# kaspanet/rusty-kaspa

Measured on NVIDIA H100. Metric: schnorr_sig_verifies_per_sec, higher is better.
Workload: dtype u32 limbs (256-bit modular integer)

## Files before the change

### __graft_entry__.py

```python
import os
import subprocess
import sys

ROOT = os.path.dirname(os.path.abspath(__file__))
CSRC = os.path.join(ROOT, "rusty_kaspa_b200", "csrc")
LIB = os.path.join(ROOT, "rusty_kaspa_b200", "libkgv.so")
NVCC_FLAGS = ["-gencode", "arch=compute_90a,code=sm_90a", "-O3", "-lineinfo", "-std=c++17", "-shared", "-Xcompiler", "-fPIC"]


def _newer(target, sources):
    if not os.path.exists(target):
        return True
    t = os.path.getmtime(target)
    return any(os.path.getmtime(s) > t for s in sources)


def _run(cmd, **kw):
    r = subprocess.run(cmd, capture_output=True, text=True, **kw)
    if r.returncode != 0:
        raise RuntimeError("command failed: %s\n%s\n%s" % (" ".join(cmd), r.stdout[-4000:], r.stderr[-4000:]))
    return r


def build():
    srcs = [os.path.join(d, f) for d, _, fs in os.walk(CSRC) for f in fs] + [os.path.join(ROOT, "include", "kgv.h")]
    units = sorted(s for s in srcs if s.endswith(".cu") or s.endswith(".cpp"))
    if _newer(LIB, srcs):
        nvcc = os.environ.get("NVCC", "nvcc")
        _run([nvcc] + NVCC_FLAGS + ["-o", LIB] + units)
    _run(["make", "-C", os.path.join(ROOT, "oracle")])
    hs = os.path.join(ROOT, "tests", "hostsim")
    for name in ("hostsim_arith", "hostsim_secp", "hostsim_comb", "hostsim_joint", "hostsim_hash", "hostsim_u3072", "hostsim_script", "hostsim_standard"):
        src, out = os.path.join(hs, name + ".cpp"), os.path.join(hs, "lib" + name + ".so")
        if os.path.exists(src) and _newer(out, [src] + srcs):
            _run(["g++", "-O2", "-std=c++17", "-shared", "-fPIC", "-o", out, src])
    sg_src, sg_lib = os.path.join(ROOT, "tools", "simgen", "kgv_simgen.cpp"), os.path.join(ROOT, "tools", "simgen", "libkgv_simgen.so")
    if os.path.exists(sg_src) and _newer(sg_lib, [sg_src]):
        _run(["g++", "-O2", "-std=c++17", "-shared", "-fPIC", "-o", sg_lib, sg_src])
    for name in ("host_mirror_test", "script_engine_mirror_test"):
        cpp_src, cpp_bin = os.path.join(ROOT, "tests", "cpp", name + ".cpp"), os.path.join(ROOT, "tests", "cpp", name)
        if os.path.exists(cpp_src) and _newer(cpp_bin, [cpp_src, LIB, os.path.join(ROOT, "include", "kgv.hpp"), os.path.join(ROOT, "include", "kgv.h")]):
            _run(["g++", "-O2", "-std=c++17", "-o", cpp_bin, cpp_src, "-L" + os.path.join(ROOT, "rusty_kaspa_b200"), "-l:libkgv.so", "-Wl,-rpath,$ORIGIN/../../rusty_kaspa_b200"])
    sys.path.insert(0, ROOT)
    import rusty_kaspa_b200
    from rusty_kaspa_b200 import _lib
    _lib.load()


def smoke():
    import ctypes
    import numpy as np
    sys.path.insert(0, ROOT)
    import rusty_kaspa_b200 as rk
    from rusty_kaspa_b200 import workload as W
    pk, msg, sig, kind = W.schnorr_triples(4096, seed=7, n_keys=256, n_nonces=256, frac_bitflip=0.05, frac_adversarial=0.05)
    ctx = rk.GpuContext(0)
    got = ctx.verify_schnorr_batch(pk, msg, sig)
    ora = ctypes.CDLL(os.path.join(ROOT, "oracle", "libkaspa_oracle.so"))
    ora.ok_secp_init()
    exp = np.zeros(len(pk), dtype=np.uint8)
    vp = lambda a: a.ctypes.data_as(ctypes.c_void_p)
    ora.ok_schnorr_verify_batch(vp(pk), vp(msg), vp(sig), ctypes.c_size_t(len(pk)), vp(exp), 4)
    assert (got == exp).all(), "GPU verdicts differ from the oracle"
    assert (got[kind == 0] == 1).all() and not (got[kind != 0] == 1).any()
    bm = ctx.status_to_bitmap(got)
    assert (bm == np.packbits((got == 1).astype(np.uint8), bitorder="little")).all()
    sys.path.insert(0, os.path.join(ROOT, "tests"))
    from rusty_kaspa_b200 import simgen
    from rusty_kaspa_b200.txbatch import build_batch
    from rusty_kaspa_b200.validator import TransactionValidator, Params
    import oracle_tx
    fk, fe, txs = simgen.funded_window(96, n_keys=64, n_nonces=64, mix=(0.5, 0.2, 0.15, 0.15))
    ents, k = [], 0
    for t in txs:
        ents.append(fe[k:k + len(t["inputs"])])
        k += len(t["inputs"])
    txs[5]["inputs"][0]["sigscript"] = txs[5]["inputs"][0]["sigscript"][:10] + bytes([txs[5]["inputs"][0]["sigscript"][10] ^ 1]) + txs[5]["inputs"][0]["sigscript"][11:]
    batch = build_batch(txs, ents)
    val = TransactionValidator(ctx, Params(storage_mass_parameter=simgen.DEFAULT_STORAGE_MASS_PARAMETER))
    res = val.validate_populated_transactions(batch, pov_daa_score=10)
    op = oracle_tx.params(coinbase_maturity=100, storage_mass_parameter=simgen.DEFAULT_STORAGE_MASS_PARAMETER)
    for i in range(len(txs)):
        e = oracle_tx.validate_populated(ora, batch, i, 10, 0, op)
        assert int(res["status"][i]) == int(e["status"]) and int(res["fee"][i]) == int(e["fee"]), (i, res[i], e)
    assert int(res["status"][5]) != 0
    from rusty_kaspa_b200.replay import DagReplayer, REPLAY_BLOCK_DTYPE
    g = simgen.FastDag(seed=3, n_keys=64, n_nonces=128, coinbase_maturity=3, mix=(0.5, 0.2, 0.15, 0.15), frac_invalid=0.1, coinbase_outputs=8)
    g.generate(24, 12)
    b, first, pov = g.take()
    arr = np.zeros(len(pov), dtype=REPLAY_BLOCK_DTYPE)
    arr["first_tx"], arr["n_txs"], arr["pov_daa_score"], arr["flags"] = first[:-1], np.diff(first), pov, 1
    rp = DagReplayer(ctx, Params(coinbase_maturity=3, storage_mass_parameter=g.C), 1 << 12)
    got_r, acc = rp.replay_window(b, arr, want_accept=True)
    ost = oracle_tx.State(ora)
    exp_r, eacc = oracle_tx.state_replay(ost, b, first, pov, oracle_tx.params(coinbase_maturity=3, storage_mass_parameter=g.C), threads=2)
    assert (got_r["status"] == exp_r["status"]).all() and (got_r["script_err"] == exp_r["script_err"]).all() and (acc == eacc).all(), "replay verdicts differ from the oracle"
    assert rp.us.count() == ost.count() and rp.us.digest() == ost.digest()
    n_replayed = len(b.txs)
    rp.close(); ost.close(); g.close()
    ctx.close()
    print("smoke ok: %d triples (%d valid), %d transactions and a replay window of %d transactions, verdicts identical to the oracle"
          % (len(pk), int((got == 1).sum()), len(txs), n_replayed))


if __name__ == "__main__":
    build()
    print("build ok")
```

### rusty_kaspa_b200/csrc/kgv_lib.cu

```cuda
#include "../../include/kgv.h"
#include "kgv_internal.h"
#include "kgv_verify.cuh"
#include "kgv_lanes.cuh"

#include <cuda_runtime.h>
#include <cstdio>
#include <algorithm>
#include <cstring>
#include <mutex>
#include <string>

using namespace kgv;

struct SmemTab {
  uint32_t* base;
  __device__ __forceinline__ void put(int e, int w, uint32_t v) { base[(e * 16 + w) * KGV_BLOCK] = v; }
  __device__ __forceinline__ uint32_t get(int e, int w) const { return base[(e * 16 + w) * KGV_BLOCK]; }
  __device__ __forceinline__ uint4* chunk(int q) const { return reinterpret_cast<uint4*>(base - threadIdx.x) + q * KGV_BLOCK + threadIdx.x; }
};
__device__ __forceinline__ void stage_fetch(SmemTab& tab, int s, const uint32_t* entry) {
#pragma unroll
  for (int c = 0; c < 4; c++) {
    const uint32_t dst = (uint32_t)__cvta_generic_to_shared(tab.chunk(4 * s + c));
    asm volatile("cp.async.cg.shared.global [%0], [%1], 16;" ::"r"(dst), "l"(entry + 4 * c) : "memory");
// ... 1 lines not shown
}
__device__ __forceinline__ void stage_commit(SmemTab&) { asm volatile("cp.async.commit_group;" ::: "memory"); }
__device__ __forceinline__ void stage_wait(SmemTab&) { asm volatile("cp.async.wait_group 7;" ::: "memory"); }
__device__ __forceinline__ void stage_get(SmemTab& tab, int s, fe& x, fe& y) {
  const uint4 a = *tab.chunk(4 * s), b = *tab.chunk(4 * s + 1), c = *tab.chunk(4 * s + 2), d = *tab.chunk(4 * s + 3);
  x.v[0] = a.x; x.v[1] = a.y; x.v[2] = a.z; x.v[3] = a.w; x.v[4] = b.x; x.v[5] = b.y; x.v[6] = b.z; x.v[7] = b.w;
  y.v[0] = c.x; y.v[1] = c.y; y.v[2] = c.z; y.v[3] = c.w; y.v[4] = d.x; y.v[5] = d.y; y.v[6] = d.z; y.v[7] = d.w;
}

__device__ __forceinline__ void ldg256(uint32_t* w, const void* p) {
  asm volatile("ld.global.nc.v4.u32 {%0,%1,%2,%3}, [%8];\n\t"
               "ld.global.nc.v4.u32 {%4,%5,%6,%7}, [%8+16];"
               : "=r"(w[0]), "=r"(w[1]), "=r"(w[2]), "=r"(w[3]), "=r"(w[4]), "=r"(w[5]), "=r"(w[6]), "=r"(w[7])
               : "l"(p));
}
__device__ __forceinline__ void ldg256_stream(uint32_t* w, const void* p) {
  asm volatile("ld.global.nc.L1::no_allocate.v4.u32 {%0,%1,%2,%3}, [%8];\n\t"
               "ld.global.nc.L1::no_allocate.v4.u32 {%4,%5,%6,%7}, [%8+16];"
               : "=r"(w[0]), "=r"(w[1]), "=r"(w[2]), "=r"(w[3]), "=r"(w[4]), "=r"(w[5]), "=r"(w[6]), "=r"(w[7])
               : "l"(p));
}

struct GLoadDev {
  __device__ __forceinline__ void operator()(fe& x, fe& y, const uint32_t* entry) const {
    ldg256(x.v, entry);
    ldg256(y.v, entry + 8);
  }
};

template <bool ALIGNED>
__device__ __forceinline__ void load_be32(uint32_t* w, const uint8_t* p) {
  if (ALIGNED) {
    ldg256_stream(w, p);
#pragma unroll
    for (int i = 0; i < 8; i++) w[i] = bswap32(w[i]);
  } else {
#pragma unroll
    for (int i = 0; i < 8; i++)
      w[i] = ((uint32_t)p[4 * i] << 24) | ((uint32_t)p[4 * i + 1] << 16) | ((uint32_t)p[4 * i + 2] << 8) | (uint32_t)p[4 * i + 3];
  }
}

__global__ void __launch_bounds__(128) k_build_gtab(uint32_t* __restrict__ gtab) {
  uint32_t t = blockIdx.x * blockDim.x + threadIdx.x;
  if (t >= 8u * 65536u) return;
  uint32_t v = t & 0xFFFFu;
  uint32_t which = t >> 16;
  uint32_t* out = gtab + (size_t)t * 16;
  if (v == 0) {
#pragma unroll
    for (int i = 0; i < 16; i++) out[i] = 0;
    return;
  }
  fe bx, by, x, y;
  gtab_base(bx, by, (int)which);
  gtab_entry(x, y, v, bx, by);
#pragma unroll
  for (int i = 0; i < 8; i++) { out[i] = x.v[i]; out[8 + i] = y.v[i]; }
}

#define KGV_KEY_RECORDS_MAX (1u << 17)
#ifndef KGV_COMB_USES
#define KGV_COMB_USES 8
#endif
enum { KGV_KEYS_INLINE = 0, KGV_KEYS_PLAIN = 1, KGV_KEYS_COMB = 2 };
__host__ __device__ __forceinline__ int key_form(uint32_t n_rec, size_t n) {
  if (n_rec > KGV_KEY_RECORDS_MAX || 2 * (size_t)n_rec > n) return KGV_KEYS_INLINE;
  return (size_t)KGV_COMB_USES * n_rec <= n ? KGV_KEYS_COMB : KGV_KEYS_PLAIN;
}

struct KeySlot {
  unsigned long long key;
  uint32_t rec, unused_;
};
struct KeyCacheView {
  const KeySlot* table;
  const uint32_t* item_slot;
  const uint32_t* recs;
  const uint32_t* n_rec;
  __device__ __forceinline__ KeySrc key_of(size_t i, size_t n) const {
    const int f = n_rec ? key_form(*n_rec, n) : KGV_KEYS_INLINE;
    if (f == KGV_KEYS_INLINE) return KeySrc{nullptr, false};
    const bool comb = f == KGV_KEYS_COMB;
    return KeySrc{recs + (size_t)(table[item_slot[i]].rec - 1) * (comb ? KGV_KJ_WORDS : KGV_KR_WORDS), comb};
  }
};

template <bool ALIGNED, bool ECDSA>
__device__ __forceinline__ void key_words(uint32_t* w, const uint8_t* pk, size_t i) {
  if (ECDSA) {
    const uint8_t* kp = pk + 33 * i;
    w[8] = kp[0];
    load_be32<false>(w, kp + 1);
  } else {
    load_be32<ALIGNED>(w, pk + 32 * i);
  }
}
__device__ __forceinline__ uint64_t key_hash(const uint32_t* w, int nw) {
  uint64_t h = 0x9E3779B97F4A7C15ull;
  for (int k = 0; k < nw; k++) {
    h = (h ^ w[k]) * 0xFF51AFD7ED558CCDull;
    h ^= h >> 32;
  }
  h ^= h >> 33; h *= 0xC4CEB9FE1A85EC53ull; h ^= h >> 33;
  return h;
}

template <bool ALIGNED, bool ECDSA>
__global__ void __launch_bounds__(256) k_key_dedup(const uint8_t* __restrict__ pk, size_t n_arg, const uint32_t* __restrict__ index,
                                                   const uint32_t* __restrict__ n_dev, KeySlot* __restrict__ table, uint32_t mask,
                                                   uint32_t* __restrict__ item_slot, uint32_t* __restrict__ rec_rep, uint32_t* n_rec) {
  const size_t n = n_dev ? (size_t)*n_dev : n_arg;
  const size_t t = (size_t)blockIdx.x * blockDim.x + threadIdx.x;
  if (t >= n || key_form(*(volatile uint32_t*)n_rec, n) == KGV_KEYS_INLINE) return;
  const size_t i = index ? index[t] : t;
  const int nw = ECDSA ? 9 : 8;
  uint32_t w[9];
  key_words<ALIGNED, ECDSA>(w, pk, i);
  const uint64_t h = key_hash(w, nw);
  const unsigned long long mine = (h & 0xFFFFFFFF00000000ull) | (uint64_t)(i + 1);
  uint32_t s = (uint32_t)h & mask;
  bool won = false;
  for (;;) {
    unsigned long long cur = atomicCAS(&table[s].key, 0ull, mine);
    if (cur == 0) { won = true; break; }
    if ((cur >> 32) == (mine >> 32)) {
      uint32_t v[9];
      key_words<ALIGNED, ECDSA>(v, pk, (uint32_t)cur - 1);
      bool eq = true;
      for (int k = 0; k < nw; k++) eq = eq && v[k] == w[k];
      if (eq) break;
    }
    s = (s + 1) & mask;
  }
  const uint32_t act = __activemask(), ball = __ballot_sync(act, won);
  const int lane = threadIdx.x & 31, leader = __ffs(act) - 1;
  uint32_t base = 0;
  if (lane == leader && ball) base = atomicAdd(n_rec, (uint32_t)__popc(ball));
  base = __shfl_sync(act, base, leader);
  if (won) {
    const uint32_t r = base + __popc(ball & ((1u << lane) - 1));
    if (key_form(r + 1, n) != KGV_KEYS_INLINE) {
      rec_rep[r] = (uint32_t)i;
      table[s].rec = r + 1;
    }
  }
  item_slot[i] = s;
}

template <bool ECDSA>
__global__ void __launch_bounds__(KGV_BLOCK, KGV_BLOCKS_PER_SM) k_key_prepare(const uint8_t* __restrict__ pk, size_t n_arg, const uint32_t* __restrict__ n_dev,
                                                                              const uint32_t* __restrict__ rec_rep, const uint32_t* __restrict__ n_rec,
                                                                              uint32_t* __restrict__ recs) {
  const size_t n = n_dev ? (size_t)*n_dev : n_arg;
  const uint32_t r = blockIdx.x * blockDim.x + threadIdx.x;
  const int f = key_form(*n_rec, n);
  if (r >= *n_rec || f == KGV_KEYS_INLINE) return;
  uint32_t w[9];
  key_words<false, ECDSA>(w, pk, rec_rep[r]);
  if (f == KGV_KEYS_COMB) {
    uint32_t* rec = recs + (size_t)r * KGV_KJ_WORDS;
    key_comb_build(rec, ECDSA ? w[8] : 2u, w);
    if (rec[KGV_KC_STATUS] == KGV_ST_VALID) key_joint_build(rec);
  } else key_rec_build(recs + (size_t)r * KGV_KR_WORDS, ECDSA ? w[8] : 2u, w);
}

template <bool ECDSA>
__device__ __forceinline__ void batch_mul(fe& r, const fe& a, const fe& b) {
  if constexpr (ECDSA) sc_mul(r.v, a.v, b.v);
  else fe_mul(r, a, b);
}
template <bool ECDSA, bool ALIGNED, bool INDEXED>
__device__ __forceinline__ void verify_body(const uint8_t* __restrict__ pk, const uint8_t* __restrict__ msg, const uint8_t* __restrict__ sig,
                                            size_t n_arg, uint8_t* __restrict__ status, const uint32_t* __restrict__ gtab,
                                            const uint32_t* __restrict__ index, const uint32_t* __restrict__ n_dev, KeyCacheView kc) {
  extern __shared__ uint32_t smem[];
  const size_t n = (INDEXED && n_dev) ? (size_t)*n_dev : n_arg;
  const size_t total = (size_t)gridDim.x * KGV_BLOCK;
  const size_t tid = (size_t)blockIdx.x * KGV_BLOCK + threadIdx.x;
  SmemTab tab{smem + threadIdx.x};
  fe X[KGV_ITEMS], Y[KGV_ITEMS], RX[KGV_ITEMS], D[KGV_ITEMS], pre[KGV_ITEMS], M[KGV_ITEMS];
  const uint32_t* KR[KGV_ITEMS];
  bool comb = false;
  uint8_t st[KGV_ITEMS];
#pragma unroll 1
  for (size_t base = 0; base < n; base += total * KGV_ITEMS) {
  fe acc;
  fe_set_u32(acc, 1);
  bool any = false;
#pragma unroll 1
  for (int j = 0; j < KGV_ITEMS; j++) {
    size_t i = base + tid + (size_t)j * total;
    st[j] = KGV_ST_INVALID;
    if (i >= n) continue;
    if (INDEXED) i = index[i];
    uint32_t pkw[9], mw[8], sw[16];
    key_words<ALIGNED, ECDSA>(pkw, pk, i);
    load_be32<ALIGNED>(mw, msg + 32 * i);
    load_be32<ALIGNED>(sw, sig + 64 * i);
    load_be32<ALIGNED>(sw + 8, sig + 64 * i + 32);
    const KeySrc key = kc.key_of(i, n);
    fe x, y, rx, d, m;
    uint8_t s1;
    if constexpr (ECDSA) s1 = ecdsa_phase1(x, y, rx.v, d.v, m.v, pkw[8], pkw, mw, sw, key);
    else s1 = schnorr_phase1(x, y, d, rx, pkw, mw, sw, tab, gtab, GLoadDev(), key);
    st[j] = s1;
    if (s1 == KGV_ST_PENDING) {
      X[j] = x; Y[j] = y; RX[j] = rx; D[j] = d;
      if constexpr (ECDSA) { M[j] = m; KR[j] = key.rec; comb = key.comb; }
      pre[j] = acc;
      batch_mul<ECDSA>(acc, acc, d);
      any = true;
    }
  }
  if (any) {
    fe inv;
    if constexpr (ECDSA) sc_inv(inv.v, acc.v);
    else fe_inv(inv, acc);
#pragma unroll 1
    for (int j = KGV_ITEMS - 1; j >= 0; j--) {
      if (st[j] != KGV_ST_PENDING) continue;
      fe di;
      batch_mul<ECDSA>(di, inv, pre[j]);
      batch_mul<ECDSA>(inv, inv, D[j]);
      if constexpr (ECDSA) st[j] = ecdsa_phase2(X[j], Y[j], RX[j].v, di.v, M[j].v, tab, gtab, GLoadDev(), KeySrc{KR[j], comb});
      else st[j] = schnorr_phase2(X[j], Y[j], di, RX[j]);
    }
  }
#pragma unroll 1
  for (int j = 0; j < KGV_ITEMS; j++) {
    size_t i = base + tid + (size_t)j * total;
    if (i < n) status[INDEXED ? index[i] : i] = st[j];
  }
  }
}

template <bool ALIGNED, bool INDEXED>
__global__ void __launch_bounds__(KGV_BLOCK, KGV_BLOCKS_PER_SM)
k_schnorr_verify(const uint8_t* __restrict__ pk, const uint8_t* __restrict__ msg, const uint8_t* __restrict__ sig, size_t n_arg,
                 uint8_t* __restrict__ status, const uint32_t* __restrict__ gtab, const uint32_t* __restrict__ index, const uint32_t* __restrict__ n_dev,
                 KeyCacheView kc) {
  verify_body<false, ALIGNED, INDEXED>(pk, msg, sig, n_arg, status, gtab, index, n_dev, kc);
}
template <bool ALIGNED, bool INDEXED>
__global__ void __launch_bounds__(KGV_BLOCK, KGV_BLOCKS_PER_SM)
k_ecdsa_verify(const uint8_t* __restrict__ pk, const uint8_t* __restrict__ msg, const uint8_t* __restrict__ sig, size_t n_arg,
               uint8_t* __restrict__ status, const uint32_t* __restrict__ gtab, const uint32_t* __restrict__ index, const uint32_t* __restrict__ n_dev,
// ... 153 lines not shown
    k_build_gtab<<<(8 * 65536) / 128, 128, 0, ctx->stream>>>(ctx->gtab);
    CK(cudaGetLastError());
    ctx->launches++;
    const int smem = KGV_BLOCK * 128 * (int)sizeof(uint32_t);
    for (const auto& kind : k_verify)
      for (const auto& form : kind)
        for (VerifyKernel k : form) CK(cudaFuncSetAttribute(k, cudaFuncAttributeMaxDynamicSharedMemorySize, smem));
    int per_sm = 0, sms = 0;
    CK(cudaOccupancyMaxActiveBlocksPerMultiprocessor(&per_sm, k_verify[0][0][1], KGV_BLOCK, smem));
    CK(cudaDeviceGetAttribute(&sms, cudaDevAttrMultiProcessorCount, device));
    ctx->resident_blocks = per_sm * sms > 0 ? per_sm * sms : 132 * KGV_BLOCKS_PER_SM;
    CK(cudaStreamSynchronize(ctx->stream));
    return KGV_OK;
  };
  int rc = body();
  if (rc != KGV_OK) {
    fprintf(stderr, "kgv_create: %s\n", ctx->err.c_str());
    delete ctx;
    return rc;
  }
  *out = ctx;
  return KGV_OK;
}

extern "C" void kgv_destroy(kgv_ctx* ctx) {
  if (!ctx) return;
  cudaSetDevice(ctx->device);
  for (auto& P : ctx->prefetch) if (P.worker.joinable()) P.worker.join();
  if (ctx->copy_stream) cudaStreamSynchronize(ctx->copy_stream);
  cudaStreamSynchronize(ctx->stream);
  if (ctx->gtab) cudaFree(ctx->gtab);
  for (uint8_t* b : {ctx->d_in, ctx->d_out, ctx->d_batch, ctx->prefetch[0].buf, ctx->prefetch[1].buf, ctx->d_scratch, ctx->d_mu, ctx->d_work, ctx->d_replay, ctx->d_keys[0], ctx->d_keys[1]})
    if (b) cudaFree(b);
  for (uint8_t* b : ctx->parked) cudaFree(b);
  for (cudaEvent_t e : ctx->ev_chunk) if (e) cudaEventDestroy(e);
  for (cudaEvent_t e : ctx->ev_time) if (e) cudaEventDestroy(e);
  if (ctx->ev_prefetch) cudaEventDestroy(ctx->ev_prefetch);
  for (auto& P : ctx->prefetch) if (P.done) cudaEventDestroy(P.done);
  if (ctx->copy_stream) cudaStreamDestroy(ctx->copy_stream);
  if (ctx->ev_fork) cudaEventDestroy(ctx->ev_fork);
  if (ctx->ev_join) cudaEventDestroy(ctx->ev_join);
  if (ctx->aux_stream) cudaStreamDestroy(ctx->aux_stream);
  if (ctx->own_stream) cudaStreamDestroy(ctx->own_stream);
  delete ctx;
}

extern "C" int kgv_set_stream(kgv_ctx* ctx, void* cuda_stream) {
  if (!ctx) return KGV_ERR_ARG;
  std::lock_guard<std::recursive_mutex> g(ctx->mu);
  ctx->stream = (cudaStream_t)cuda_stream;
  return KGV_OK;
}

extern "C" int kgv_reset_stream(kgv_ctx* ctx) {
  if (!ctx) return KGV_ERR_ARG;
  std::lock_guard<std::recursive_mutex> g(ctx->mu);
  ctx->stream = ctx->own_stream;
  return KGV_OK;
}

extern "C" int kgv_synchronize(kgv_ctx* ctx) {
  if (!ctx) return KGV_ERR_ARG;
  std::lock_guard<std::recursive_mutex> g(ctx->mu);
  CK(cudaSetDevice(ctx->device));
  CK(cudaStreamSynchronize(ctx->stream));
  if (!ctx->parked.empty()) {
    CK(cudaStreamSynchronize(ctx->aux_stream));
    if (ctx->copy_stream) CK(cudaStreamSynchronize(ctx->copy_stream));
    for (uint8_t* p : ctx->parked) cudaFree(p);
    ctx->parked.clear();
  }
  return KGV_OK;
}

extern "C" const char* kgv_last_error(const kgv_ctx* ctx) { return ctx ? ctx->err.c_str() : "null context"; }
extern "C" uint64_t kgv_launch_count(const kgv_ctx* ctx) { return ctx ? ctx->launches : 0; }

static int key_cache_launch(kgv_ctx* ctx, const uint8_t* dpk, size_t n, bool ecdsa, bool aligned, cudaStream_t st, const uint32_t* index,
                            const uint32_t* n_dev, KeyCacheView* kc) {
  uint32_t slots = 64;
  while (slots < 2 * n) slots <<= 1;
  const uint32_t cap = (uint32_t)(n / 2 < KGV_KEY_RECORDS_MAX ? n / 2 : KGV_KEY_RECORDS_MAX);
  const size_t cap_comb = n / KGV_COMB_USES < KGV_KEY_RECORDS_MAX ? n / KGV_COMB_USES : KGV_KEY_RECORDS_MAX;
  const size_t rec_bytes = std::max((size_t)cap * KGV_KR_WORDS, cap_comb * KGV_KJ_WORDS) * 4;
  const size_t o_tab = 256, o_item = o_tab + (size_t)slots * sizeof(KeySlot);
  const size_t o_rep = (o_item + n * 4 + 255) & ~(size_t)255, o_rec = (o_rep + (size_t)cap * 4 + 255) & ~(size_t)255;
  int rc = kgv_reserve(ctx, &ctx->d_keys[ecdsa], &ctx->d_keys_cap[ecdsa], o_rec + rec_bytes);
  if (rc) return rc;
  uint8_t* K = ctx->d_keys[ecdsa];
  uint32_t* n_rec = (uint32_t*)K;
  KeySlot* table = (KeySlot*)(K + o_tab);
  uint32_t *item_slot = (uint32_t*)(K + o_item), *rec_rep = (uint32_t*)(K + o_rep), *recs = (uint32_t*)(K + o_rec);
  CK(cudaMemsetAsync(K, 0, o_item, st));
  const unsigned gd = (unsigned)((n + 255) / 256);
  const auto dedup = ecdsa ? k_key_dedup<false, true> : aligned ? k_key_dedup<true, false> : k_key_dedup<false, false>;
  dedup<<<gd, 256, 0, st>>>(dpk, n, index, n_dev, table, slots - 1, item_slot, rec_rep, n_rec);
  CK(cudaGetLastError());
  ctx->launches++;
  if (cap) {
    const unsigned gp = (cap + KGV_BLOCK - 1) / KGV_BLOCK;
    const auto prepare = ecdsa ? k_key_prepare<true> : k_key_prepare<false>;
    prepare<<<gp, KGV_BLOCK, 0, st>>>(dpk, n, n_dev, rec_rep, n_rec, recs);
    CK(cudaGetLastError());
    ctx->launches++;
  }
  *kc = KeyCacheView{table, item_slot, recs, n_rec};
  return KGV_OK;
}

int kgv_launch_verify(kgv_ctx* ctx, const uint8_t* dpk, const uint8_t* dmsg, const uint8_t* dsig, size_t n, uint8_t* dst, bool ecdsa,
                      cudaStream_t st, const uint32_t* index, const uint32_t* n_dev) {
  if (n == 0) return KGV_OK;
  if (n >= 0x7FFFFFFFu) return fail_arg(ctx, "verify launch of 2^31 or more items");
  const int smem = KGV_BLOCK * 128 * (int)sizeof(uint32_t);
  size_t want = (n + KGV_BLOCK - 1) / KGV_BLOCK;
  unsigned blocks = (unsigned)(want < (size_t)ctx->resident_blocks ? want : (size_t)ctx->resident_blocks);
  bool aligned = (((uintptr_t)dmsg | (uintptr_t)dsig | (ecdsa ? 0 : (uintptr_t)dpk)) & 31) == 0;
  KeyCacheView kc{};
  const bool key_cache = n > (size_t)ctx->resident_blocks * KGV_BLOCK;
  if (key_cache) {
    int rc = key_cache_launch(ctx, dpk, n, ecdsa, aligned, st, index, n_dev, &kc);
    if (rc) return rc;
  }
  if (!index) {
    auto& lv = ctx->last_verify[ecdsa];
    lv.n = n; lv.blocks = blocks; lv.key_cache = key_cache; lv.stream = st;
  }
  k_verify[ecdsa][index != nullptr][aligned]<<<blocks, KGV_BLOCK, smem, st>>>(dpk, dmsg, dsig, n, dst, ctx->gtab, index, n_dev, kc);
  CK(cudaGetLastError());
  ctx->launches++;
  return KGV_OK;
}

static int verify_common(kgv_ctx* ctx, const uint8_t* pk, size_t pk_stride, const uint8_t* msg, const uint8_t* sig, size_t n,
                         uint8_t* status, bool ecdsa) {
  if (!ctx) return KGV_ERR_ARG;
  std::lock_guard<std::recursive_mutex> g(ctx->mu);
  if (n == 0) return KGV_OK;
  if (!pk || !msg || !sig || !status) return fail_arg(ctx, "null buffer");
  CK(cudaSetDevice(ctx->device));
  int dev = kgv_ptr_is_device(pk);
  if (kgv_ptr_is_device(msg) != dev || kgv_ptr_is_device(sig) != dev || kgv_ptr_is_device(status) != dev)
    return fail_arg(ctx, "all buffers of one call must be host pointers or all device pointers");
  const uint8_t *dpk = pk, *dmsg = msg, *dsig = sig;
  uint8_t* dst = status;
  if (!dev) {
    size_t off_msg = (pk_stride * n + 255) & ~(size_t)255;
    size_t off_sig = off_msg + 32 * n;
    int rc = kgv_reserve(ctx, &ctx->d_in, &ctx->d_in_cap, off_sig + 64 * n);
    if (rc) return rc;
    rc = kgv_reserve(ctx, &ctx->d_out, &ctx->d_out_cap, n);
    if (rc) return rc;
    dpk = ctx->d_in; dmsg = ctx->d_in + off_msg; dsig = ctx->d_in + off_sig; dst = ctx->d_out;
    const size_t chunk = (size_t)ctx->resident_blocks * KGV_BLOCK * KGV_ITEMS;
    if (n >= 2 * chunk && (n + chunk - 1) / chunk <= 32) {
      CK(cudaEventRecord(ctx->ev_fork, ctx->stream));
      CK(cudaStreamWaitEvent(ctx->aux_stream, ctx->ev_fork, 0));
      size_t c = 0;
      for (size_t a = 0; a < n; a += chunk, c++) {
        const size_t m = n - a < chunk ? n - a : chunk;
        if (!ctx->ev_chunk[c]) CK(cudaEventCreateWithFlags(&ctx->ev_chunk[c], cudaEventDisableTiming));
        CK(cudaMemcpyAsync(ctx->d_in + pk_stride * a, pk + pk_stride * a, pk_stride * m, cudaMemcpyHostToDevice, ctx->aux_stream));
        CK(cudaMemcpyAsync(ctx->d_in + off_msg + 32 * a, msg + 32 * a, 32 * m, cudaMemcpyHostToDevice, ctx->aux_stream));
        CK(cudaMemcpyAsync(ctx->d_in + off_sig + 64 * a, sig + 64 * a, 64 * m, cudaMemcpyHostToDevice, ctx->aux_stream));
        CK(cudaEventRecord(ctx->ev_chunk[c], ctx->aux_stream));
        CK(cudaStreamWaitEvent(ctx->stream, ctx->ev_chunk[c], 0));
        int rc2 = kgv_launch_verify(ctx, dpk + pk_stride * a, dmsg + 32 * a, dsig + 64 * a, m, dst + a, ecdsa, ctx->stream);
// ... 144 lines not shown
```

### rusty_kaspa_b200/csrc/kgv_secp.cuh

```cuda
#pragma once
#include "kgv_arith.cuh"

namespace kgv {

#define KGV_N_LIMBS {0xD0364141u, 0xBFD25E8Cu, 0xAF48A03Bu, 0xBAAEDCE6u, 0xFFFFFFFEu, 0xFFFFFFFFu, 0xFFFFFFFFu, 0xFFFFFFFFu}
#define KGV_BETA_LIMBS {0x719501EEu, 0xC1396C28u, 0x12F58995u, 0x9CF04975u, 0xAC3434E9u, 0x6E64479Eu, 0x657C0710u, 0x7AE96A2Bu}
#define KGV_G1_LIMBS {0x45DBB031u, 0xE893209Au, 0x71E8CA7Fu, 0x3DAA8A14u, 0x9284EB15u, 0xE86C90E4u, 0xA7D46BCDu, 0x3086D221u}
#define KGV_G2_LIMBS {0x8AC47F71u, 0x1571B4AEu, 0x9DF506C6u, 0x221208ACu, 0x0ABFE4C4u, 0x6F547FA9u, 0x010E8828u, 0xE4437ED6u}
#define KGV_A1_LIMBS {0x9284EB15u, 0xE86C90E4u, 0xA7D46BCDu, 0x3086D221u, 0u}
#define KGV_MB1_LIMBS {0x0ABFE4C3u, 0x6F547FA9u, 0x010E8828u, 0xE4437ED6u, 0u}
#define KGV_A2_LIMBS {0x9D44CFD8u, 0x57C1108Du, 0xA8E2F3F6u, 0x14CA50F7u, 1u}

struct gej {
  fe x, y, z;
  bool inf;
};

struct NoTrace {
  KGV_HD void operator()(int , const uint32_t* , int ) const {}
};

KGV_HD bool sc_ge_n(const uint32_t* a) {
  const uint32_t n[8] = KGV_N_LIMBS;
  return !lt8(a, n);
// ... 278 lines not shown
    if (hout) fe_set_u32(*hout, 1);
    return false;
  }
  fe z1z1, u2, s2, h, rr, t;
  fe_sqr(z1z1, r.z);
  fe_mul(u2, bx, z1z1);
  fe_mul(t, r.z, z1z1);
  fe_mul(s2, by, t);
  fe_sub(h, u2, r.x);
  fe_sub(rr, s2, r.y);
  if (fe_is_zero(h)) {
    if (fe_is_zero(rr)) return true;
    if (hout) fe_set_u32(*hout, 1);
    r.inf = true;
    return false;
  }
  if (hout) *hout = h;
  fe hh, hhh, v;
  fex w;
  fe_sqr(hh, h);
  fe_mul(hhh, hh, h);
  fe_mul(v, r.x, hh);
  fe_mul(r.z, r.z, h);
  fe_sqr(t, rr);
  fex_set(w, t); fex_sub(w, hhh); fex_sub(w, v); fex_sub(w, v);
  fe_fold(r.x, w);
  fe_sub(t, v, r.x);
  fe_mul(t, rr, t);
  fe_mul(hhh, r.y, hhh);
  fe_sub(r.y, t, hhh);
  return false;
}

#if defined(__CUDACC__)
struct gej_h { gej r; fe h; };
static __device__ __noinline__ gej_h gej_point_call(gej r, fe bx, fe by, int n) {
  gej_h o;
  if (n == 0 && gej_add_ge_body(r, bx, by, &o.h)) {
    fe_dbl(o.h, r.y);
    n = 1;
  }
#pragma unroll 1
  for (int i = 0; i < n; i++) gej_double_body(r);
  o.r = r;
  return o;
}
KGV_HD void gej_double_n(gej& r, int n) {
  if (!r.inf) r = gej_point_call(r, r.x, r.y, n).r;
}
KGV_HD void gej_add_ge(gej& r, const fe& bx, const fe& by, fe* hout = nullptr) {
  gej_h o = gej_point_call(r, bx, by, 0);
  r = o.r;
  if (hout) *hout = o.h;
}
#else
KGV_HD void gej_double_n(gej& r, int n) {
  if (r.inf) return;
  for (int i = 0; i < n; i++) gej_double_body(r);
}
KGV_HD void gej_add_ge(gej& r, const fe& bx, const fe& by, fe* hout = nullptr) {
  if (gej_add_ge_body(r, bx, by, hout)) {
    if (hout) fe_dbl(*hout, r.y);
    gej_double_n(r, 1);
  }
}
#endif
KGV_HD void gej_double(gej& r) { gej_double_n(r, 1); }

KGV_HD bool ge_lift_x(fe& y, const fe& x, bool odd) {
  fe t, c;
  fe_sqr(t, x);
  fe_mul(t, t, x);
  fe_set_u32(c, 7);
  fe_add(c, t, c);
  if (!fe_sqrt(y, c)) return false;
  fe_normalize(y);
  if (((y.v[0] & 1u) != 0) != odd) {
    fe_neg(y, y);
    fe_normalize(y);
  }
  return true;
}

template <class Tab>
KGV_HD void build_odd_table(Tab& tab, fe& zs, const fe& px, const fe& py) {
  gej d;
  d.x = px; d.y = py; fe_set_u32(d.z, 1); d.inf = false;
  gej_double(d);
  fe zd2, zd3;
  fe_sqr(zd2, d.z);
  fe_mul(zd3, zd2, d.z);
  gej t;
  fe_mul(t.x, px, zd2);
  fe_mul(t.y, py, zd3);
  fe_set_u32(t.z, 1);
  t.inf = false;
  fe H[7];
#pragma unroll
  for (int w = 0; w < 8; w++) { tab.put(0, w, t.x.v[w]); tab.put(0, 8 + w, t.y.v[w]); }
#pragma unroll
  for (int j = 1; j < 8; j++) {
    gej_add_ge(t, d.x, d.y, &H[j - 1]);
#pragma unroll
    for (int w = 0; w < 8; w++) { tab.put(j, w, t.x.v[w]); tab.put(j, 8 + w, t.y.v[w]); }
  }
  fe acc = H[6];
#pragma unroll
  for (int j = 6; j >= 0; j--) {
    if (j < 6) fe_mul(acc, acc, H[j]);
    fe a2, a3, ex, ey;
    fe_sqr(a2, acc);
    fe_mul(a3, a2, acc);
#pragma unroll
    for (int w = 0; w < 8; w++) { ex.v[w] = tab.get(j, w); ey.v[w] = tab.get(j, 8 + w); }
    fe_mul(ex, ex, a2);
    fe_mul(ey, ey, a3);
#pragma unroll
    for (int w = 0; w < 8; w++) { tab.put(j, w, ex.v[w]); tab.put(j, 8 + w, ey.v[w]); }
  }
  fe_mul(zs, t.z, d.z);
}

template <class Tab, class GLoad, class Trace = NoTrace>
KGV_HD void ecmult_double(gej& R, const fe& zs, const uint32_t* kP, const uint32_t* kG, Tab& tab, const uint32_t* gtab, GLoad gload,
                          Trace trace = Trace()) {
  const fe beta = {KGV_BETA_LIMBS};
  uint32_t m1[5], m2[5], h1[5], h2[5];
  bool neg1, neg2, fix1, fix2;
  glv_split(m1, neg1, m2, neg2, kP);
  recode_signed_odd(h1, fix1, m1);
  recode_signed_odd(h2, fix2, m2);
  trace(10, m1, 5); trace(11, m2, 5);
  { uint32_t f[4] = {neg1, neg2, fix1, fix2}; trace(12, f, 4); }
  trace(13, zs.v, 8);
  { uint32_t e0[16]; for (int w = 0; w < 16; w++) e0[w] = tab.get(7, w); trace(14, e0, 16); }
  fe zs2, zs3;
  fe_sqr(zs2, zs);
  fe_mul(zs3, zs2, zs);

  R.inf = true;
  fe_set_zero(R.x); fe_set_zero(R.y); fe_set_zero(R.z);
  for (int i = 32; i >= 0; i--) {
    if (i != 32) gej_double_n(R, 4);
    uint32_t idx; bool dn;
    fe ex, ey;
    recoded_digit(h1, i, idx, dn);
#pragma unroll
    for (int w = 0; w < 8; w++) { ex.v[w] = tab.get(idx, w); ey.v[w] = tab.get(idx, 8 + w); }
    if (dn != neg1) fe_neg(ey, ey);
    gej_add_ge(R, ex, ey);
    recoded_digit(h2, i, idx, dn);
#pragma unroll
    for (int w = 0; w < 8; w++) { ex.v[w] = tab.get(idx, w); ey.v[w] = tab.get(idx, 8 + w); }
    fe_mul(ex, ex, beta);
    if (dn != neg2) fe_neg(ey, ey);
    gej_add_ge(R, ex, ey);
    if ((i & 3) == 0 && i < 32) {
      int w16 = i >> 2;
      uint32_t dlo = (kG[w16 >> 1] >> ((w16 & 1) * 16)) & 0xFFFFu;
      uint32_t dhi = (kG[4 + (w16 >> 1)] >> ((w16 & 1) * 16)) & 0xFFFFu;
      if (dlo) {
        gload(ex, ey, gtab + (size_t)dlo * 16);
        fe_mul(ex, ex, zs2);
        fe_mul(ey, ey, zs3);
        gej_add_ge(R, ex, ey);
      }
      if (dhi) {
        gload(ex, ey, gtab + ((size_t)4 * 65536 + dhi) * 16);
        fe_mul(ex, ex, zs2);
        fe_mul(ey, ey, zs3);
        gej_add_ge(R, ex, ey);
      }
    }
  }
  trace(15, R.x.v, 8); trace(16, R.y.v, 8); trace(17, R.z.v, 8);
  if (fix1) {
    fe ex, ey;
#pragma unroll
    for (int w = 0; w < 8; w++) { ex.v[w] = tab.get(0, w); ey.v[w] = tab.get(0, 8 + w); }
    if (!neg1) fe_neg(ey, ey);
    gej_add_ge(R, ex, ey);
  }
  if (fix2) {
    fe ex, ey;
#pragma unroll
    for (int w = 0; w < 8; w++) { ex.v[w] = tab.get(0, w); ey.v[w] = tab.get(0, 8 + w); }
    fe_mul(ex, ex, beta);
    if (!neg2) fe_neg(ey, ey);
    gej_add_ge(R, ex, ey);
  }
}

// ... 179 lines not shown
```

### rusty_kaspa_b200/csrc/kgv_verify.cuh

```cuda
#pragma once
#include "kgv_secp.cuh"
#include "kgv_sha256.cuh"

namespace kgv {

enum : uint8_t { KGV_ST_INVALID = 0, KGV_ST_VALID = 1, KGV_ST_PK_PARSE = 2, KGV_ST_SIG_PARSE = 3 };

KGV_HD bool fe_words_lt_p(const uint32_t* v) {
  const uint32_t p[8] = {KGV_P0, KGV_P1, 0xFFFFFFFFu, 0xFFFFFFFFu, 0xFFFFFFFFu, 0xFFFFFFFFu, 0xFFFFFFFFu, 0xFFFFFFFFu};
  return lt8(v, p);
}

#define KGV_ST_PENDING 0xFFu

KGV_HD bool key_lift(fe& x, fe& y, uint32_t tag, const uint32_t* pkw) {
  if (tag != 2u && tag != 3u) return false;
  limbs_from_be_words(x.v, pkw);
  if (!fe_words_lt_p(x.v)) return false;
  return ge_lift_x(y, x, tag == 3u);
}

#define KGV_KR_ZS 128
#define KGV_KR_STATUS 136
#define KGV_KR_WORDS 140
#define KGV_KC_STATUS 512
#define KGV_KC_WORDS 528
#define KGV_KJ_JOINT KGV_KC_WORDS
#define KGV_KJ_WORDS (KGV_KJ_JOINT + 4 * 32 * 16)

struct RecTab {
  uint32_t* rec;
  KGV_HD void put(int e, int w, uint32_t v) { rec[e * 16 + w] = v; }
  KGV_HD uint32_t get(int e, int w) const { return rec[e * 16 + w]; }
};
KGV_HD void ldg128(uint32_t* w, const uint32_t* p) {
#ifdef __CUDA_ARCH__
  asm volatile("ld.global.nc.v4.u32 {%0,%1,%2,%3}, [%4];" : "=r"(w[0]), "=r"(w[1]), "=r"(w[2]), "=r"(w[3]) : "l"(p));
#else
  for (int i = 0; i < 4; i++) w[i] = p[i];
#endif
}
KGV_HD void fe_ld(fe& x, const uint32_t* p) {
#ifdef __CUDA_ARCH__
  const uint4 a = reinterpret_cast<const uint4*>(p)[0], b = reinterpret_cast<const uint4*>(p)[1];
  x.v[0] = a.x; x.v[1] = a.y; x.v[2] = a.z; x.v[3] = a.w; x.v[4] = b.x; x.v[5] = b.y; x.v[6] = b.z; x.v[7] = b.w;
#else
  for (int w = 0; w < 8; w++) x.v[w] = p[w];
#endif
}
KGV_HD void fe_st(uint32_t* p, const fe& x) {
#ifdef __CUDA_ARCH__
  reinterpret_cast<uint4*>(p)[0] = make_uint4(x.v[0], x.v[1], x.v[2], x.v[3]);
  reinterpret_cast<uint4*>(p)[1] = make_uint4(x.v[4], x.v[5], x.v[6], x.v[7]);
#else
  for (int w = 0; w < 8; w++) p[w] = x.v[w];
#endif
}
template <class Tab>
KGV_HD void key_rec_load(Tab& tab, fe& zs, const uint32_t* rec) {
#pragma unroll 1
  for (int e = 0; e < 8; e++) {
    uint32_t w[16];
#pragma unroll
    for (int q = 0; q < 4; q++) ldg128(w + 4 * q, rec + 16 * e + 4 * q);
#pragma unroll
    for (int q = 0; q < 16; q++) tab.put(e, q, w[q]);
  }
  ldg128(zs.v, rec + KGV_KR_ZS);
  ldg128(zs.v + 4, rec + KGV_KR_ZS + 4);
}
KGV_HD void key_rec_build(uint32_t* rec, uint32_t tag, const uint32_t* pkw) {
  fe x, y, zs;
  uint8_t st = KGV_ST_PK_PARSE;
  if (key_lift(x, y, tag, pkw)) {
    RecTab tab{rec};
    build_odd_table(tab, zs, x, y);
#pragma unroll
    for (int w = 0; w < 8; w++) rec[KGV_KR_ZS + w] = zs.v[w];
    st = KGV_ST_VALID;
  }
  rec[KGV_KR_STATUS] = st;
}
KGV_HD void key_comb_build(uint32_t* rec, uint32_t tag, const uint32_t* pkw) {
  fe x, y;
  uint8_t st = KGV_ST_PK_PARSE;
  if (key_lift(x, y, tag, pkw)) {
    gej b;
    b.x = x; b.y = y; fe_set_u32(b.z, 1); b.inf = false;
    fe zs[4], pre[4], inv;
#pragma unroll 1
    for (int t = 0; t < 4; t++) {
      if (t) gej_double_n(b, 32);
      RecTab tab{rec + 128 * t};
      fe z;
      build_odd_table(tab, z, b.x, b.y);
      fe_mul(zs[t], z, b.z);
      if (t) fe_mul(pre[t], pre[t - 1], zs[t]);
      else pre[0] = zs[0];
    }
    fe_inv(inv, pre[3]);
#pragma unroll 1
    for (int t = 3; t >= 0; t--) {
      fe zi, zi2, zi3;
      if (t) {
        fe_mul(zi, inv, pre[t - 1]);
        fe_mul(inv, inv, zs[t]);
      } else {
// ... 11 lines not shown
        fe_mul(ey, ey, zi3);
        fe_st(en, ex);
        fe_st(en + 8, ey);
      }
    }
    st = KGV_ST_VALID;
  }
  rec[KGV_KC_STATUS] = st;
}

KGV_HD void key_joint_build(uint32_t* rec) {
  const fe beta = {KGV_BETA_LIMBS};
  uint32_t* jt = rec + KGV_KJ_JOINT;
#pragma unroll 1
  for (int t = 0; t < 4; t++) {
#pragma unroll 1
    for (int j = 0; j < 4; j++) {
      fe bx;
      fe_ld(bx, rec + 16 * (8 * t + j));
      fe_mul(bx, bx, beta);
      fe_st(jt + 16 * (32 * t + 3 - j), bx);
    }
  }
  fe acc;
  fe_set_u32(acc, 1);
#pragma unroll 1
  for (int ta = 0; ta < 16; ta++) {
    const int t = ta >> 2, a = ta & 3;
    fe xa;
    fe_ld(xa, rec + 16 * (8 * t + a));
#pragma unroll 1
    for (int j = 0; j < 4; j++) {
      fe bx, d;
      fe_ld(bx, jt + 16 * (32 * t + 3 - j));
      fe_sub(d, bx, xa);
      fe_mul(acc, acc, d);
      fe_st(jt + 16 * (32 * t + 8 * a + j + 4), acc);
    }
  }
  fe inv;
  fe_inv(inv, acc);
#pragma unroll 1
  for (int ta = 15; ta >= 0; ta--) {
    const int t = ta >> 2, a = ta & 3;
    fe xa, ya;
    fe_ld(xa, rec + 16 * (8 * t + a));
    fe_ld(ya, rec + 16 * (8 * t + a) + 8);
#pragma unroll 1
    for (int j = 3; j >= 0; j--) {
      const int p = 4 * ta + j, q = p - 1;
      fe bx, yb, d, di;
      fe_ld(bx, jt + 16 * (32 * t + 3 - j));
      fe_ld(yb, rec + 16 * (8 * t + j) + 8);
      if (p) {
        fe pre;
        fe_ld(pre, jt + 16 * (32 * (q >> 4) + 8 * ((q >> 2) & 3) + (q & 3) + 4));
        fe_sub(d, bx, xa);
        fe_mul(di, inv, pre);
        fe_mul(inv, inv, d);
      } else {
        di = inv;
      }
#pragma unroll 1
      for (int sgn = 0; sgn < 2; sgn++) {
        fe l, x3, y3, t1;
        if (sgn) fe_neg(t1, yb);
        else t1 = yb;
        fe_sub(t1, t1, ya);
        fe_mul(l, t1, di);
        fe_sqr(x3, l);
        fe_sub(x3, x3, xa);
        fe_sub(x3, x3, bx);
        fe_sub(t1, xa, x3);
        fe_mul(y3, l, t1);
        fe_sub(y3, y3, ya);
        uint32_t* en = jt + 16 * (32 * t + 8 * a + (sgn ? 3 - j : j + 4));
        fe_st(en, x3);
        fe_st(en + 8, y3);
      }
    }
  }
}

struct KeySrc {
  const uint32_t* rec;
  bool comb;
};
KGV_HD bool key_rec_valid(const KeySrc& key) { return key.rec[key.comb ? KGV_KC_STATUS : KGV_KR_STATUS] == KGV_ST_VALID; }
template <class Tab, class GLoad, class Trace = NoTrace>
KGV_HD void ecmult_key(gej& R, fe& zt, const KeySrc& key, const fe& px, const fe& py, const uint32_t* kP, const uint32_t* kG, Tab& tab,
                       const uint32_t* gtab, GLoad gload, Trace trace = Trace()) {
  fe zs;
  if (key.comb) {
    ecmult_joint(R, kP, kG, key.rec, key.rec + KGV_KJ_JOINT, tab, gtab, gload);
  } else {
    if (key.rec) key_rec_load(tab, zs, key.rec);
    else build_odd_table(tab, zs, px, py);
    ecmult_double(R, zs, kP, kG, tab, gtab, gload, trace);
  }
  if (R.inf) return;
  if (key.comb) zt = R.z;
  else fe_mul(zt, R.z, zs);
}

template <class Tab, class GLoad, class Trace = NoTrace>
KGV_HD uint8_t schnorr_phase1(fe& X, fe& Y, fe& zt, fe& rx, const uint32_t* pkw, const uint32_t* mw, const uint32_t* sigw, Tab& tab,
                              const uint32_t* gtab, GLoad gload, const KeySrc& key, Trace trace = Trace()) {
  fe px, py;
  if (key.rec) {
    if (!key_rec_valid(key)) return KGV_ST_PK_PARSE;
  } else {
    limbs_from_be_words(px.v, pkw);
    if (!fe_words_lt_p(px.v)) return KGV_ST_PK_PARSE;
    trace(1, px.v, 8);
    if (!ge_lift_x(py, px, false)) return KGV_ST_PK_PARSE;
    trace(2, py.v, 8);
  }
  limbs_from_be_words(rx.v, sigw);
  if (!fe_words_lt_p(rx.v)) return KGV_ST_INVALID;
  uint32_t s[8], e[8], k[8], ew[8];
  limbs_from_be_words(s, sigw + 8);
  if (sc_ge_n(s)) return KGV_ST_INVALID;
  bip340_challenge(ew, sigw, pkw, mw);
#pragma unroll
  for (int i = 0; i < 8; i++) e[7 - i] = ew[i];
  sc_reduce_once(e);
  sc_neg(k, e);
  trace(3, e, 8); trace(4, k, 8); trace(5, s, 8);
  gej R;
  ecmult_key(R, zt, key, px, py, k, s, tab, gtab, gload, trace);
  { uint32_t f[1] = {R.inf}; trace(18, f, 1); }
  if (R.inf) return KGV_ST_INVALID;
  trace(19, R.x.v, 8); trace(20, R.y.v, 8); trace(21, R.z.v, 8);
  X = R.x;
  Y = R.y;
  return KGV_ST_PENDING;
}
template <class Trace = NoTrace>
KGV_HD uint8_t schnorr_phase2(const fe& X, const fe& Y, const fe& zi, const fe& rx, Trace trace = Trace()) {
  fe zi2, ax, ay;
  fe_sqr(zi2, zi);
  fe_mul(ax, X, zi2);
  fe_mul(ay, Y, zi2);
  fe_mul(ay, ay, zi);
  fe_normalize(ay);
  fe_normalize(ax);
  trace(22, ax.v, 8); trace(23, ay.v, 8);
  if (ay.v[0] & 1u) return KGV_ST_INVALID;
  bool eq = true;
#pragma unroll
  for (int i = 0; i < 8; i++) eq = eq && (ax.v[i] == rx.v[i]);
  return eq ? KGV_ST_VALID : KGV_ST_INVALID;
}
template <class Tab, class GLoad, class Trace = NoTrace>
KGV_HD uint8_t schnorr_verify_core(const uint32_t* pkw, const uint32_t* mw, const uint32_t* sigw, Tab& tab, const uint32_t* gtab,
                                   GLoad gload, Trace trace = Trace(), KeySrc key = KeySrc{nullptr, false}) {
  fe X, Y, zt, rx, zi;
  uint8_t st = schnorr_phase1(X, Y, zt, rx, pkw, mw, sigw, tab, gtab, gload, key, trace);
  if (st != KGV_ST_PENDING) return st;
  fe_inv(zi, zt);
  return schnorr_phase2(X, Y, zi, rx, trace);
}

KGV_HD uint8_t ecdsa_phase1(fe& qx, fe& qy, uint32_t* r, uint32_t* s, uint32_t* m, uint32_t tag, const uint32_t* pkw, const uint32_t* mw,
                            const uint32_t* sigw, const KeySrc& key) {
  if (key.rec) {
    if (!key_rec_valid(key)) return KGV_ST_PK_PARSE;
  } else if (!key_lift(qx, qy, tag, pkw)) {
    return KGV_ST_PK_PARSE;
  }
  limbs_from_be_words(r, sigw);
  limbs_from_be_words(s, sigw + 8);
  if (sc_ge_n(r) || sc_ge_n(s)) return KGV_ST_SIG_PARSE;
  limbs_from_be_words(m, mw);
  sc_reduce_once(m);
  if (sc_is_high(s)) return KGV_ST_INVALID;
  if (is_zero8(r) || is_zero8(s)) return KGV_ST_INVALID;
// ... 81 lines not shown
```

Measured before the change: 61.63 million.

## Build joint key records directly without intermediate comb table

Replaces the two-step key preparation (full comb record then joint table) with a single joint-record builder. It builds small 4-entry odd-multiple tables for four shifted base points and batches every required inversion into one field inversion. The record shrinks to the point coordinates, a status word and the joint table, cutting prep work and record memory. A separate launch bound for the prep kernel is also added; the builder keeps large per-thread arrays, so register spills are a risk.

```diff
diff --git a/__graft_entry__.py b/__graft_entry__.py
--- a/__graft_entry__.py
+++ b/__graft_entry__.py
@@ -30,7 +30,7 @@
         _run([nvcc] + NVCC_FLAGS + ["-o", LIB] + units)
     _run(["make", "-C", os.path.join(ROOT, "oracle")])
     hs = os.path.join(ROOT, "tests", "hostsim")
-    for name in ("hostsim_arith", "hostsim_secp", "hostsim_comb", "hostsim_joint", "hostsim_hash", "hostsim_u3072", "hostsim_script", "hostsim_standard"):
+    for name in ("hostsim_arith", "hostsim_secp", "hostsim_comb", "hostsim_joint", "hostsim_joint_record", "hostsim_hash", "hostsim_u3072", "hostsim_script", "hostsim_standard"):
         src, out = os.path.join(hs, name + ".cpp"), os.path.join(hs, "lib" + name + ".so")
         if os.path.exists(src) and _newer(out, [src] + srcs):
             _run(["g++", "-O2", "-std=c++17", "-shared", "-fPIC", "-o", out, src])
diff --git a/rusty_kaspa_b200/csrc/kgv_lib.cu b/rusty_kaspa_b200/csrc/kgv_lib.cu
--- a/rusty_kaspa_b200/csrc/kgv_lib.cu
+++ b/rusty_kaspa_b200/csrc/kgv_lib.cu
@@ -107,7 +107,7 @@
     const int f = n_rec ? key_form(*n_rec, n) : KGV_KEYS_INLINE;
     if (f == KGV_KEYS_INLINE) return KeySrc{nullptr, false};
     const bool comb = f == KGV_KEYS_COMB;
-    return KeySrc{recs + (size_t)(table[item_slot[i]].rec - 1) * (comb ? KGV_KJ_WORDS : KGV_KR_WORDS), comb};
+    return KeySrc{recs + (size_t)(table[item_slot[i]].rec - 1) * (comb ? KGV_JR_WORDS : KGV_KR_WORDS), comb};
   }
 };
 
@@ -173,8 +173,11 @@
   item_slot[i] = s;
 }
 
+#ifndef KGV_PREP_BLOCKS_PER_SM
+#define KGV_PREP_BLOCKS_PER_SM 5
+#endif
 template <bool ECDSA>
-__global__ void __launch_bounds__(KGV_BLOCK, KGV_BLOCKS_PER_SM) k_key_prepare(const uint8_t* __restrict__ pk, size_t n_arg, const uint32_t* __restrict__ n_dev,
+__global__ void __launch_bounds__(KGV_BLOCK, KGV_PREP_BLOCKS_PER_SM) k_key_prepare(const uint8_t* __restrict__ pk, size_t n_arg, const uint32_t* __restrict__ n_dev,
                                                                               const uint32_t* __restrict__ rec_rep, const uint32_t* __restrict__ n_rec,
                                                                               uint32_t* __restrict__ recs) {
   const size_t n = n_dev ? (size_t)*n_dev : n_arg;
@@ -183,11 +186,8 @@
   if (r >= *n_rec || f == KGV_KEYS_INLINE) return;
   uint32_t w[9];
   key_words<false, ECDSA>(w, pk, rec_rep[r]);
-  if (f == KGV_KEYS_COMB) {
-    uint32_t* rec = recs + (size_t)r * KGV_KJ_WORDS;
-    key_comb_build(rec, ECDSA ? w[8] : 2u, w);
-    if (rec[KGV_KC_STATUS] == KGV_ST_VALID) key_joint_build(rec);
-  } else key_rec_build(recs + (size_t)r * KGV_KR_WORDS, ECDSA ? w[8] : 2u, w);
+  if (f == KGV_KEYS_COMB) key_joint_record_build(recs + (size_t)r * KGV_JR_WORDS, ECDSA ? w[8] : 2u, w);
+  else key_rec_build(recs + (size_t)r * KGV_KR_WORDS, ECDSA ? w[8] : 2u, w);
 }
 
 template <bool ECDSA>
@@ -507,7 +507,7 @@
   while (slots < 2 * n) slots <<= 1;
   const uint32_t cap = (uint32_t)(n / 2 < KGV_KEY_RECORDS_MAX ? n / 2 : KGV_KEY_RECORDS_MAX);
   const size_t cap_comb = n / KGV_COMB_USES < KGV_KEY_RECORDS_MAX ? n / KGV_COMB_USES : KGV_KEY_RECORDS_MAX;
-  const size_t rec_bytes = std::max((size_t)cap * KGV_KR_WORDS, cap_comb * KGV_KJ_WORDS) * 4;
+  const size_t rec_bytes = std::max((size_t)cap * KGV_KR_WORDS, cap_comb * KGV_JR_WORDS) * 4;
   const size_t o_tab = 256, o_item = o_tab + (size_t)slots * sizeof(KeySlot);
   const size_t o_rep = (o_item + n * 4 + 255) & ~(size_t)255, o_rec = (o_rep + (size_t)cap * 4 + 255) & ~(size_t)255;
   int rc = kgv_reserve(ctx, &ctx->d_keys[ecdsa], &ctx->d_keys_cap[ecdsa], o_rec + rec_bytes);
diff --git a/rusty_kaspa_b200/csrc/kgv_secp.cuh b/rusty_kaspa_b200/csrc/kgv_secp.cuh
--- a/rusty_kaspa_b200/csrc/kgv_secp.cuh
+++ b/rusty_kaspa_b200/csrc/kgv_secp.cuh
@@ -384,8 +384,9 @@
   return true;
 }
 
-template <class Tab>
+template <int NE = 8, class Tab>
 KGV_HD void build_odd_table(Tab& tab, fe& zs, const fe& px, const fe& py) {
+  static_assert(NE >= 2 && NE <= 8, "build_odd_table: 2 to 8 entries");
   gej d;
   d.x = px; d.y = py; fe_set_u32(d.z, 1); d.inf = false;
   gej_double(d);
@@ -397,19 +398,19 @@
   fe_mul(t.y, py, zd3);
   fe_set_u32(t.z, 1);
   t.inf = false;
-  fe H[7];
+  fe H[NE - 1];
 #pragma unroll
   for (int w = 0; w < 8; w++) { tab.put(0, w, t.x.v[w]); tab.put(0, 8 + w, t.y.v[w]); }
 #pragma unroll
-  for (int j = 1; j < 8; j++) {
+  for (int j = 1; j < NE; j++) {
     gej_add_ge(t, d.x, d.y, &H[j - 1]);
 #pragma unroll
     for (int w = 0; w < 8; w++) { tab.put(j, w, t.x.v[w]); tab.put(j, 8 + w, t.y.v[w]); }
   }
-  fe acc = H[6];
-#pragma unroll
-  for (int j = 6; j >= 0; j--) {
-    if (j < 6) fe_mul(acc, acc, H[j]);
+  fe acc = H[NE - 2];
+#pragma unroll
+  for (int j = NE - 2; j >= 0; j--) {
+    if (j < NE - 2) fe_mul(acc, acc, H[j]);
     fe a2, a3, ex, ey;
     fe_sqr(a2, acc);
     fe_mul(a3, a2, acc);
diff --git a/rusty_kaspa_b200/csrc/kgv_verify.cuh b/rusty_kaspa_b200/csrc/kgv_verify.cuh
--- a/rusty_kaspa_b200/csrc/kgv_verify.cuh
+++ b/rusty_kaspa_b200/csrc/kgv_verify.cuh
@@ -23,6 +23,10 @@
 #define KGV_KR_ZS 128
 #define KGV_KR_STATUS 136
 #define KGV_KR_WORDS 140
+#define KGV_JR_P 0
+#define KGV_JR_STATUS 16
+#define KGV_JR_JOINT 32
+#define KGV_JR_WORDS (KGV_JR_JOINT + 4 * 32 * 16)
 #define KGV_KC_STATUS 512
 #define KGV_KC_WORDS 528
 #define KGV_KJ_JOINT KGV_KC_WORDS
@@ -200,17 +204,120 @@
   }
 }
 
+struct FeTab {
+  fe* x;
+  fe* y;
+  KGV_HD void put(int e, int w, uint32_t v) {
+    if (w < 8) x[e].v[w] = v;
+    else y[e].v[w - 8] = v;
+  }
+  KGV_HD uint32_t get(int e, int w) const { return w < 8 ? x[e].v[w] : y[e].v[w - 8]; }
+};
+KGV_HD void joint_table_build(uint32_t* jt, const fe& px, const fe& py) {
+  const fe beta = {KGV_BETA_LIMBS};
+  fe ex[16], ey[16], eb[16];
+  fe dn[64], pre[64];
+  fe zs[4], zp[5];
+  gej b;
+  b.x = px; b.y = py; fe_set_u32(b.z, 1); b.inf = false;
+#pragma unroll 1
+  for (int t = 0; t < 4; t++) {
+    if (t) gej_double_n(b, 32);
+    FeTab tab{ex + 4 * t, ey + 4 * t};
+    fe z;
+    build_odd_table<4>(tab, z, b.x, b.y);
+    fe_mul(zs[t], z, b.z);
+#pragma unroll 1
+    for (int e = 0; e < 4; e++) fe_mul(eb[4 * t + e], ex[4 * t + e], beta);
+  }
+  fe acc;
+#pragma unroll 1
+  for (int p = 0; p < 64; p++) {
+    const int t = p >> 4, a = (p >> 2) & 3, j = p & 3;
+    fe d;
+    fe_sub(d, eb[4 * t + j], ex[4 * t + a]);
+    if (p) fe_mul(acc, acc, d);
+    else acc = d;
+    dn[p] = d;
+    pre[p] = acc;
+  }
+  zp[0] = acc;
+#pragma unroll 1
+  for (int t = 0; t < 4; t++) {
+    fe_mul(acc, acc, zs[t]);
+    zp[t + 1] = acc;
+  }
+  fe inv;
+  fe_inv(inv, acc);
+#pragma unroll 1
+  for (int t = 3; t >= 0; t--) {
+    fe zi, zi2, zi3;
+    fe_mul(zi, inv, zp[t]);
+    fe_mul(inv, inv, zs[t]);
+    fe_sqr(zi2, zi);
+    fe_mul(zi3, zi2, zi);
+    fe_sqr(zs[t], zs[t]);
+#pragma unroll 1
+    for (int e = 4 * t; e < 4 * t + 4; e++) {
+      fe_mul(ex[e], ex[e], zi2);
+      fe_mul(ey[e], ey[e], zi3);
+      fe_mul(eb[e], eb[e], zi2);
+    }
+  }
+#pragma unroll 1
+  for (int p = 63; p >= 0; p--) {
+    const int t = p >> 4, a = (p >> 2) & 3, j = p & 3;
+    fe di;
+    if (p) {
+      fe_mul(di, inv, pre[p - 1]);
+      fe_mul(inv, inv, dn[p]);
+    } else {
+      di = inv;
+    }
+    fe_mul(di, di, zs[t]);
+    const fe xa = ex[4 * t + a], ya = ey[4 * t + a], bx = eb[4 * t + j], yb = ey[4 * t + j];
+#pragma unroll 1
+    for (int sgn = 0; sgn < 2; sgn++) {
+      fe l, x3, y3, t1;
+      if (sgn) fe_neg(t1, yb);
+      else t1 = yb;
+      fe_sub(t1, t1, ya);
+      fe_mul(l, t1, di);
+      fe_sqr(x3, l);
+      fe_sub(x3, x3, xa);
+      fe_sub(x3, x3, bx);
+      fe_sub(t1, xa, x3);
+      fe_mul(y3, l, t1);
+      fe_sub(y3, y3, ya);
+      uint32_t* en = jt + 16 * (32 * t + 8 * a + (sgn ? 3 - j : j + 4));
+      fe_st(en, x3);
+      fe_st(en + 8, y3);
+    }
+  }
+}
+KGV_HD void key_joint_record_build(uint32_t* rec, uint32_t tag, const uint32_t* pkw) {
+  fe x, y;
+  uint8_t st = KGV_ST_PK_PARSE;
+  if (key_lift(x, y, tag, pkw)) {
+    fe_st(rec + KGV_JR_P, x);
+    fe_st(rec + KGV_JR_P + 8, y);
+    joint_table_build(rec + KGV_JR_JOINT, x, y);
+    st = KGV_ST_VALID;
+  }
+  rec[KGV_JR_STATUS] = st;
+}
+
 struct KeySrc {
   const uint32_t* rec;
   bool comb;
 };
-KGV_HD bool key_rec_valid(const KeySrc& key) { return key.rec[key.comb ? KGV_KC_STATUS : KGV_KR_STATUS] == KGV_ST_VALID; }
+KGV_HD bool key_rec_valid(const KeySrc& key) { return key.rec[key.comb ? KGV_JR_STATUS : KGV_KR_STATUS] == KGV_ST_VALID; }
 template <class Tab, class GLoad, class Trace = NoTrace>
 KGV_HD void ecmult_key(gej& R, fe& zt, const KeySrc& key, const fe& px, const fe& py, const uint32_t* kP, const uint32_t* kG, Tab& tab,
                        const uint32_t* gtab, GLoad gload, Trace trace = Trace()) {
   fe zs;
   if (key.comb) {
-    ecmult_joint(R, kP, kG, key.rec, key.rec + KGV_KJ_JOINT, tab, gtab, gload);
+    ecmult_joint(R, kP, kG, key.rec + KGV_JR_P, key.rec + KGV_JR_JOINT, tab, gtab, gload);
   } else {
     if (key.rec) key_rec_load(tab, zs, key.rec);
     else build_odd_table(tab, zs, px, py);
```

Result: faster. 64.54 million, median of 6 (+4.7%).
